# tarepan/ForwardTacotron

Measured on AMD Instinct MI355X. Metric: mel-frames/sec at batch=64 LJSpeech shapes (ForwardTacotron.generate, B*T_mel per s), higher is better.
Workload: dtype fp32; 1 GPU; c3: ForwardTacotron generate, batch=64 per GPU, phoneme lengths U{50..200}; global_batch=64, T_phonemes=200, T_mel=1368, parallelism=dp1

## Files before the change

### forwardtacotron_amd/csrc/gemm.hip

```cpp
#include "common.h"

namespace {

constexpr int BM = 128;
constexpr int BN = 128;
constexpr int BK = 16;
constexpr int LDS_STRIDE = 20;
constexpr int MAX_GROUPS = 16;

enum { EPI_CONV = 0, EPI_HIGHWAY = 1 };

struct GemmGroup {
  const float *w;
  const __bf16 *w3;
  const float *colscale;
  int Kpad;
  const float *bias;
  const float *scale;
  const float *shift;
  int N, k, pad, Ktot;
  int ycol0;
  int ntiles;
  int tile0;
};
// ... 654 lines not shown
  const int tid = threadIdx.x;
  const int lane = tid & 63, wave = tid >> 6;
  const int fr = lane & 15, fs = lane >> 4;

  const float *arow[2];
  int at[2];
  bool aok[2];
#pragma unroll
  for (int mi = 0; mi < 2; ++mi) {
    const int m = m0 + wave * 32 + mi * 16 + fr;
    aok[mi] = m < p.M;
    const int mm = aok[mi] ? m : 0;
    const int b = mm / p.To;
    at[mi] = mm - b * p.To;
    arow[mi] = p.x + (int64_t)b * p.T * p.x_stride;
  }
  int nk = (G.Ktot + X6_BK - 1) / X6_BK;
  int kc0 = 0;
  if (p.split > 1) {
    kc0 = blockIdx.y * p.kc_per;
    nk = min(nk - kc0, p.kc_per);
  }
  int kk = kc0 * X6_BK + 8 * fs, tj = kk / p.Cin, tc = kk - tj * p.Cin;
  struct ARaw {
    f32x4 v[2][2];
    f32x4 u[MAXPOOL ? 2 : 1][2];
    unsigned okm;
  };
  auto loadA = [&](ARaw &r) {
    const bool kok = kk < G.Ktot;
    unsigned okm = 0;
#pragma unroll
    for (int mi = 0; mi < 2; ++mi) {
      const int ts = at[mi] + tj - G.pad;
      const bool ok = kok && aok[mi] && ts >= 0 && ts < p.T;
      const float *src = arow[mi] + (int64_t)(ok ? ts : 0) * p.x_stride + (ok ? tc : 0);
      r.v[mi][0] = *(const f32x4 *)src;
      r.v[mi][1] = *(const f32x4 *)(src + 4);
      if constexpr (MAXPOOL) {
        const float *sp = src - ((ok && ts > 0) ? p.x_stride : 0);
        r.u[mi][0] = *(const f32x4 *)sp;
        r.u[mi][1] = *(const f32x4 *)(sp + 4);
      }
      okm |= (unsigned)ok << mi;
    }
    r.okm = okm;
    kk += X6_BK;
    tc += X6_BK;
#pragma unroll
    for (int w = 0; w < 2; ++w) {
      const bool wrap = tc >= p.Cin;
      tc -= wrap ? p.Cin : 0;
      tj += wrap;
    }
  };
  float amax = 0.f;
  auto splitA = [&](const ARaw &r, frag (&a)[2][H3 ? 2 : 3]) {
#pragma unroll
    for (int mi = 0; mi < 2; ++mi) {
      f32x4 v0 = r.v[mi][0], v1 = r.v[mi][1];
      if constexpr (MAXPOOL) {
        v0 = fmax4(v0, r.u[mi][0]);
        v1 = fmax4(v1, r.u[mi][1]);
      }
      const bool ok = (r.okm >> mi) & 1u;
      v0 = sel4(ok, v0);
      v1 = sel4(ok, v1);
      if constexpr (H3) {
        amax = fmaxf(amax, fmaxf(fmaxf(fabsf(v0.x), fabsf(v0.y)), fmaxf(fabsf(v0.z), fabsf(v0.w))));
        amax = fmaxf(amax, fmaxf(fmaxf(fabsf(v1.x), fabsf(v1.y)), fmaxf(fabsf(v1.z), fabsf(v1.w))));
        f16x4 l1, l2, h1, h2;
        split2h(v0, l1, l2);
        split2h(v1, h1, h2);
        a[mi][0] = __builtin_shufflevector(l1, h1, 0, 1, 2, 3, 4, 5, 6, 7);
        a[mi][1] = __builtin_shufflevector(l2, h2, 0, 1, 2, 3, 4, 5, 6, 7);
      } else {
        bf16x4 l1, l2, l3, h1, h2, h3;
        split3(v0, l1, l2, l3);
        split3(v1, h1, h2, h3);
        a[mi][0] = __builtin_shufflevector(l1, h1, 0, 1, 2, 3, 4, 5, 6, 7);
        a[mi][1] = __builtin_shufflevector(l2, h2, 0, 1, 2, 3, 4, 5, 6, 7);
        a[mi][2] = __builtin_shufflevector(l3, h3, 0, 1, 2, 3, 4, 5, 6, 7);
      }
    }
  };

  typedef unsigned u32x4 __attribute__((ext_vector_type(4)));
  const __bf16 *bsrc[6];
  int boff[6];
#pragma unroll
  for (int i = 0; i < 6; ++i) {
    const int idx = tid + 256 * i;
    const int pc = idx >> 9, rem = idx & 511, nl = rem >> 2, seg = rem & 3;
    const int n = n0 + nl < G.N ? n0 + nl : G.N - 1;
    bsrc[i] = G.w3 + ((int64_t)pc * G.N + n) * G.Kpad + kc0 * X6_BK + seg * 8;
    boff[i] = pc * X6_PIECE + nl * X6_STRIDE + seg * 8;
  }
  const int kb_last = (nk - 1) * X6_BK;
  int kb = 0;
  auto loadB = [&](u32x4 (&rb)[6]) {
    const int o = kb < kb_last ? kb : kb_last;
#pragma unroll
    for (int i = 0; i < 6; ++i) rb[i] = *(const u32x4 *)(bsrc[i] + o);
    kb += X6_BK;
  };
  auto storeB = [&](const u32x4 (&rb)[6], int buf) {
#pragma unroll
    for (int i = 0; i < 6; ++i) *(u32x4 *)(lds + buf * 3 * X6_PIECE + boff[i]) = rb[i];
  };

  f32x4 acc[2][8];
#pragma unroll
  for (int mi = 0; mi < 2; ++mi)
#pragma unroll
    for (int ni = 0; ni < 8; ++ni) acc[mi][ni] = (f32x4){0.f, 0.f, 0.f, 0.f};

  auto mfma_chunk = [&](const frag (&a)[2][H3 ? 2 : 3], int buf) {
    const __bf16 *cur = lds + buf * 3 * X6_PIECE;
#pragma unroll
    for (int ni = 0; ni < 8; ++ni) {
      frag b[3];
#pragma unroll
      for (int pc = 0; pc < 3; ++pc)
        b[pc] = *(const frag *)(cur + pc * X6_PIECE + (ni * 16 + fr) * X6_STRIDE + 8 * fs);
#pragma unroll
      for (int mi = 0; mi < 2; ++mi) {
        f32x4 c = acc[mi][ni];
        if constexpr (H3) {
          c = mma16(a[mi][1], b[2], c);
          c = mma16(a[mi][0], b[1], c);
          c = mma16(a[mi][0], b[0], c);
        } else {
          c = mma16(a[mi][2], b[0], c);
          c = mma16(a[mi][1], b[1], c);
          c = mma16(a[mi][0], b[2], c);
          c = mma16(a[mi][1], b[0], c);
          c = mma16(a[mi][0], b[1], c);
          c = mma16(a[mi][0], b[0], c);
        }
        acc[mi][ni] = c;
      }
    }
  };

  constexpr bool DEEP = H3;
  ARaw ra0, ra1;
  u32x4 rb[6];
  loadA(ra0);
  loadB(rb);
  if constexpr (DEEP) loadA(ra1);
  storeB(rb, 0);
  loadB(rb);
  __syncthreads();
  auto step = [&](int kc, ARaw &ras) {
    frag a[2][H3 ? 2 : 3];
    splitA(ras, a);
    loadA(ras);
    if (kc + 1 < nk) storeB(rb, (kc + 1) & 1);
    loadB(rb);
    mfma_chunk(a, kc & 1);
    __syncthreads();
  };
  for (int kc = 0; kc < nk; kc += 2) {
    step(kc, ra0);
    if (kc + 1 >= nk) break;
    step(kc + 1, DEEP ? ra1 : ra0);
  }

  if constexpr (H3) {
    bool bad = !(amax <= 65504.f);
#pragma unroll
    for (int ni = 0; ni < 8; ++ni) {
      const int col = n0 + ni * 16 + fr;
      const float cs = G.colscale[col < G.N ? col : G.N - 1];
#pragma unroll
      for (int mi = 0; mi < 2; ++mi)
#pragma unroll
        for (int i = 0; i < 4; ++i) {
          const int row = m0 + wave * 32 + mi * 16 + 4 * fs + i;
          bad |= col < G.N && row >= 0 && row < p.M && !__builtin_isfinite(acc[mi][ni][i]);
          acc[mi][ni][i] *= cs;
        }
    }
    if (bad && p.status) atomicOr(p.status, 1u);
  }

  const int er = 4 * fs;
  if (p.split > 1) {
    float *part = p.part + (size_t)blockIdx.y * p.M * G.N;
#pragma unroll
    for (int ni = 0; ni < 8; ++ni) {
      const int col = n0 + ni * 16 + fr;
      if (col >= G.N) continue;
#pragma unroll
      for (int mi = 0; mi < 2; ++mi)
#pragma unroll
        for (int i = 0; i < 4; ++i) {
          const int row = m0 + wave * 32 + mi * 16 + er + i;
          if (row < p.M) part[(size_t)row * G.N + col] = acc[mi][ni][i];
        }
    }
    return;
  }
  if constexpr (EPI == EPI_CONV) {
#pragma unroll
    for (int ni = 0; ni < 8; ++ni) {
      const int col = n0 + ni * 16 + fr;
      if (col >= G.N) continue;
      const float bias = G.bias ? G.bias[col] : 0.f;
      const float sc = G.scale ? G.scale[col] : 1.f;
      const float sh = G.scale ? G.shift[col] : 0.f;
#pragma unroll
      for (int mi = 0; mi < 2; ++mi)
#pragma unroll
        for (int i = 0; i < 4; ++i) {
          const int row = m0 + wave * 32 + mi * 16 + er + i;
          if (row >= p.M) continue;
          float v = acc[mi][ni][i];
          if (G.bias) v += bias;
          if (p.relu) v = fmaxf(v, 0.f);
          if (G.scale) v = v * sc + sh;
          if (p.residual) v += p.residual[(int64_t)row * p.res_stride + col];
          if (p.y) p.y[(int64_t)row * p.y_stride + G.ycol0 + col] = v;
          if (p.yt) {
            const int b = row / p.To, t = row - b * p.To;
            p.yt[((int64_t)b * p.yt_channels + G.ycol0 + col) * p.To + t] = v;
          }
        }
    }
  } else {
#pragma unroll
    for (int q = 0; q < 2; ++q)
#pragma unroll
      for (int h = 0; h < 2; ++h) {
        if (n0 + q * 64 >= G.N) continue;
        const int ni = 4 * q + h;
        const int col = n0 / 2 + q * 32 + h * 16 + fr;
        const float b1 = p.b1[col], b2 = p.b2[col];
#pragma unroll
        for (int mi = 0; mi < 2; ++mi)
#pragma unroll
          for (int i = 0; i < 4; ++i) {
            const int row = m0 + wave * 32 + mi * 16 + er + i;
            if (row >= p.M) continue;
            const float x1 = acc[mi][ni][i] + b1;
            const float x2 = acc[mi][ni + 2][i] + b2;
            const float g = ftmi_sigmoid(x2);
            const float xin = p.x[(int64_t)row * p.x_stride + col];
            p.y[(int64_t)row * p.y_stride + col] = highway_mix(g, x1, xin);
          }
      }
  }
}

constexpr int SL_BM = 256;
constexpr int SL_BN = 128;
constexpr int SL_MAXK = 16;
constexpr int SL_SR = SL_BM + SL_MAXK - 1;
constexpr int SL_P = 48;
constexpr int SL_ZROW = SL_SR;
constexpr int SL_AIMG = (SL_SR + 1) * SL_P;
constexpr int SL_BIMG = SL_BN * SL_P;
constexpr int SL_TP = SL_BN + 4;

__device__ __forceinline__ void slab_tile(int bid, int MT, int VT, int band, int &mt, int &v8) {
  if (MT < 8) {
    mt = bid % MT;
    v8 = bid / MT;
    return;
  }
  const int x = bid & 7, s8 = bid >> 3;
  if (band <= 0 || band >= VT) {
    const int q8 = s8 / VT;
    mt = q8 * 8 + x;
    v8 = s8 - q8 * VT;
    return;
  }
  const int MTx = (MT + 7) >> 3;
  const int per = MTx * band, b = s8 / per, rem = s8 - b * per;
  const int cbn = min(band, VT - b * band);
  const int lr = rem / cbn;
  mt = lr * 8 + x;
  v8 = b * band + (rem - lr * cbn);
  if (lr >= MTx) mt = MT;
}


template <int EPI, int NTHR>
__device__ __forceinline__ void slab_epilogue(const GemmParams &p, const GemmGroup &G,
                                              float *tile, int m0, int n0, int tid) {
  const int rows = min(SL_BM, p.M - m0);
  const int ncols = min(SL_BN, G.N - n0);

  if (p.split > 1) {
    float *part = p.part + (size_t)blockIdx.y * p.M * G.N;
    for (int idx = tid; idx < SL_BM * (SL_BN / 4); idx += NTHR) {
      const int r = idx >> 5, c = (idx & 31) * 4;
      if (r < rows && c < ncols)
        *(f32x4 *)(part + (size_t)(m0 + r) * G.N + n0 + c) = *(const f32x4 *)(tile + r * SL_TP + c);
    }
    return;
  }
  if constexpr (EPI == EPI_CONV) {
    if (p.pool_out) {
      for (int idx = tid; idx < SL_BM * (SL_BN / 4); idx += NTHR) {
        const int r = idx >> 5, c = (idx & 31) * 4;
        if (r >= rows || c >= ncols) continue;
        const int col = n0 + c;
        f32x4 v = *(const f32x4 *)(tile + r * SL_TP + c);
        if (G.bias) v += *(const f32x4 *)(G.bias + col);
        if (p.relu) v = fmax4(v, (f32x4){0.f, 0.f, 0.f, 0.f});
        if (G.scale) v = v * *(const f32x4 *)(G.scale + col) + *(const f32x4 *)(G.shift + col);
        *(f32x4 *)(tile + r * SL_TP + c) = v;
      }
      __syncthreads();
      float ymax = 0.f;
      for (int idx = tid; idx < SL_BM * (SL_BN / 4); idx += NTHR) {
        const int r = idx >> 5, c = (idx & 31) * 4;
        if (r == 0 || r >= rows || c >= ncols) continue;
        const int row = m0 + r, col = n0 + c;
        f32x4 v = *(const f32x4 *)(tile + r * SL_TP + c);
        if (row % p.T > 0) v = fmax4(v, *(const f32x4 *)(tile + (r - 1) * SL_TP + c));
        if (p.y_split_c) {
          ymax = fmaxf(ymax, fmaxf(fmaxf(fabsf(v.x), fabsf(v.y)), fmaxf(fabsf(v.z), fabsf(v.w))));
          f16x4 h, t;
          split2h(v, h, t);
          _Float16 *yr = (_Float16 *)(p.y + (int64_t)row * p.y_stride) + G.ycol0 + col;
          *(f16x4 *)yr = h;
          *(f16x4 *)(yr + p.y_split_c) = t;
        } else {
          *(f32x4 *)(p.y + (int64_t)row * p.y_stride + G.ycol0 + col) = v;
        }
      }
      if (!(ymax <= 65504.f) && p.status) atomicOr(p.status, 1u);
      return;
    }
    for (int idx = tid; idx < SL_BM * (SL_BN / 4); idx += NTHR) {
      const int r = idx >> 5, c = (idx & 31) * 4;
      if (r >= rows || c >= ncols) continue;
      const int row = m0 + r, col = n0 + c;
      f32x4 v = *(const f32x4 *)(tile + r * SL_TP + c);
      if (G.bias) v += *(const f32x4 *)(G.bias + col);
      if (p.relu) v = fmax4(v, (f32x4){0.f, 0.f, 0.f, 0.f});
      if (G.scale) v = v * *(const f32x4 *)(G.scale + col) + *(const f32x4 *)(G.shift + col);
      if (p.residual) v += *(const f32x4 *)(p.residual + (int64_t)row * p.res_stride + col);
      if (p.y) *(f32x4 *)(p.y + (int64_t)row * p.y_stride + G.ycol0 + col) = v;
      if (p.yt) *(f32x4 *)(tile + r * SL_TP + c) = v;
    }
    if (p.yt) {
      __syncthreads();
      for (int idx = tid; idx < SL_BM * SL_BN; idx += NTHR) {
        const int r = idx & (SL_BM - 1), c = idx / SL_BM;
        if (r >= rows || c >= ncols) continue;
        const int row = m0 + r, b = row / p.To, t = row - b * p.To;
        p.yt[((int64_t)b * p.yt_channels + G.ycol0 + n0 + c) * p.To + t] = tile[r * SL_TP + c];
      }
    }
  } else {
    for (int idx = tid; idx < SL_BM * (SL_BN / 8); idx += NTHR) {
      const int r = idx >> 4, o = (idx & 15) * 4, q = o >> 5, h = o & 31;
      if (r >= rows || q * 64 >= ncols) continue;
      const int row = m0 + r, col = n0 / 2 + o;
      const f32x4 x1 = *(const f32x4 *)(tile + r * SL_TP + q * 64 + h) + *(const f32x4 *)(p.b1 + col);
      const f32x4 x2 = *(const f32x4 *)(tile + r * SL_TP + q * 64 + 32 + h) + *(const f32x4 *)(p.b2 + col);
      const f32x4 xin = *(const f32x4 *)(p.x + (int64_t)row * p.x_stride + col);
      f32x4 out;
#pragma unroll
      for (int e = 0; e < 4; ++e) {
        const float g = ftmi_sigmoid(x2[e]);
        out[e] = highway_mix(g, x1[e], xin[e]);
      }
      *(f32x4 *)(p.y + (int64_t)row * p.y_stride + col) = out;
    }
  }
}

template <int EPI, bool MAXPOOL, bool WS>
__global__ __launch_bounds__(WS ? 768 : 512, 1) void conv_gemm_slab_kernel(const GemmParams p) {
  constexpr int NTHR = WS ? 768 : 512;
  constexpr int NSTG = WS ? 256 : 512;
  constexpr int SL_ASLOTS = (SL_SR * 8 + NSTG - 1) / NSTG;
  constexpr int SL_BSLOTS = 1024 / NSTG;
  __shared__ __attribute__((aligned(16))) _Float16 lds[2 * 2 * SL_AIMG + 2 * 2 * SL_BIMG];
  static_assert(SL_BM * SL_TP * 4 <= sizeof(lds), "epilogue tile");
  _Float16 *const lds_a = lds;
  _Float16 *const lds_b = lds + 2 * 2 * SL_AIMG;
  typedef unsigned u32x4 __attribute__((ext_vector_type(4)));
  typedef unsigned u32x2 __attribute__((ext_vector_type(2)));
  const int TS = p.pool_out ? SL_BM - 1 : SL_BM;
  const int MT = (p.M + TS - 1) / TS, NT = p.g[0].ntiles, VT = p.ngroups * NT;
  int mt, v8;
  slab_tile(blockIdx.x, MT, VT, p.band, mt, v8);
  const int gi = v8 / NT, nt = v8 - gi * NT;
  if (mt >= MT) return;
  const GemmGroup &G = p.g[gi];
  const int m0 = p.pool_out ? mt * TS - 1 : mt * SL_BM, n0 = nt * SL_BN;
  const int k = G.k, pad = G.pad, Cin = p.Cin;

  const int tid = threadIdx.x, lane = tid & 63, wave = tid >> 6;
  const int wm = wave & 3, wn = (wave >> 2) & 1;
  const int fr = lane & 15, fs = lane >> 4;
  const bool is_mma = !WS || wave < 8;
  const bool is_stg = !WS || wave >= 8;
  const int stid = WS ? tid - 512 : tid;
// ... 2420 lines not shown
#else
    if (q.T == q.M)
      hipLaunchKernelGGL((conv_gemm_skinny_kernel<false, true, 0, true>), grid, block, 0, s, q);
    else
      hipLaunchKernelGGL((conv_gemm_skinny_kernel<false, true>), grid, block, 0, s, q);
#endif
  } else {
    dim3 grid(MT * q.ngroups * NT, q.split), block(512);
    const bool nm = q.T == q.M;
    if (maxpool && nm)
      hipLaunchKernelGGL((conv_gemm_skinny_kernel<true, false, 0, true>), grid, block, 0, s, q);
    else if (maxpool)
      hipLaunchKernelGGL(conv_gemm_skinny_kernel<true>, grid, block, 0, s, q);
    else if (nm)
      hipLaunchKernelGGL((conv_gemm_skinny_kernel<false, false, 0, true>), grid, block, 0, s, q);
    else
      hipLaunchKernelGGL(conv_gemm_skinny_kernel<false>, grid, block, 0, s, q);
  }
  FTMI_CHECK_LAUNCH();
  if (q.force_part) {
    const int64_t n_el = (int64_t)q.M * (q.g[0].N / 2);
    const int eb = (int)((n_el + 255) / 256 < 2048 ? (n_el + 255) / 256 : 2048);
    hipLaunchKernelGGL(skinny_highway_finish_kernel, dim3(eb), dim3(256), 0, s, q);
    FTMI_CHECK_LAUNCH();
  } else if (q.split > 1) {
    const int64_t n_el = (int64_t)q.M * q.g[0].N;
    if (q.split >= 8) {
      const int eb = (int)((n_el + 63) / 64 < 2048 ? (n_el + 63) / 64 : 2048);
      hipLaunchKernelGGL(skinny_finish_kernel<4>, dim3(eb, q.ngroups), dim3(256), 0, s, q);
    } else {
      const int eb = (int)((n_el + 255) / 256 < 1024 ? (n_el + 255) / 256 : 1024);
      hipLaunchKernelGGL(skinny_finish_kernel<1>, dim3(eb, q.ngroups), dim3(256), 0, s, q);
    }
    FTMI_CHECK_LAUNCH();
  }
  return FTMI_OK;
}

static bool bank_halves_ok(const GemmParams &p) {
  if (p.M <= 0 || p.M > 128 || p.ngroups < 2 || p.ngroups % 2 || p.To != p.T) return false;
  if (p.Cin % 64 || p.Cin > 2 * BH_MAXCH * 32) return false;
  if (!p.y || p.yt || p.residual || p.x_split || p.pool_out || p.y_split_c) return false;
  if (!p.tile_cnt || !p.part || p.g[0].N % 16) return false;
  const int units = (p.ngroups / 2) * (p.g[0].N / 16);
  if (units % 8 || units * 8 > FTMI_BANK_COUNTERS) return false;
  for (int i = 0; i < p.ngroups; ++i)
    if (p.g[i].k != p.ngroups - i || p.g[i].N != p.g[0].N || !p.g[i].w3 || !p.g[i].colscale)
      return false;
  return true;
}

static int64_t bank_halves_floats(int M, int K, int N) {
  const int MI = M <= 64 ? 4 : 8;
  return (int64_t)(K / 2) * (N / 16) * 2 * (2 * MI * 64) * 4;
}

static int launch_bank_halves(const GemmParams &p, hipStream_t s) {
  const int units = (p.ngroups / 2) * (p.g[0].N / 16);
  const dim3 grid(2 * units), block(512);
  const int nch = p.Cin / 64;
  const bool prenet = p.ngroups == 16 && p.g[0].N == 256 && nch == 4;
#ifdef FTMI_DIAG
  const char *dg = getenv("FTMI_BANK_HALVES_DIAG");
  const int diag = dg && prenet && p.M > 64 ? atoi(dg) : 0;
  if (diag && p.wimg) {
    switch (diag) {
#define FTMI_BH_DIAG(D_)                                                                          \
  case D_:                                                                                        \
    hipLaunchKernelGGL((conv_bank_halves_kernel<8, 4, D_, 16, 16, true>), grid, block, 0, s, p);    \
    break;
      FTMI_BH_DIAG(1) FTMI_BH_DIAG(2) FTMI_BH_DIAG(3) FTMI_BH_DIAG(4) FTMI_BH_DIAG(16)
      FTMI_BH_DIAG(18) FTMI_BH_DIAG(32) FTMI_BH_DIAG(128) FTMI_BH_DIAG(256) FTMI_BH_DIAG(512)
#undef FTMI_BH_DIAG
      default:
        hipLaunchKernelGGL((conv_bank_halves_kernel<8, 4, 0, 16, 16, true>), grid, block, 0, s, p);
    }
    FTMI_CHECK_LAUNCH();
    return FTMI_OK;
  }
#endif
#define FTMI_BH_NCH(MI_, PK_)                                                                            \
  switch (nch) {                                                                                         \
    case 1: hipLaunchKernelGGL((conv_bank_halves_kernel<MI_, 1, 0, 0, 0, PK_>), grid, block, 0, s, p); break; \
    case 2: hipLaunchKernelGGL((conv_bank_halves_kernel<MI_, 2, 0, 0, 0, PK_>), grid, block, 0, s, p); break; \
    case 3: hipLaunchKernelGGL((conv_bank_halves_kernel<MI_, 3, 0, 0, 0, PK_>), grid, block, 0, s, p); break; \
    default: hipLaunchKernelGGL((conv_bank_halves_kernel<MI_, 4, 0, 0, 0, PK_>), grid, block, 0, s, p);       \
  }
  if (p.wimg) {
    if (p.M <= 64) {
      FTMI_BH_NCH(4, true)
    } else if (prenet && p.T == p.M) {
      hipLaunchKernelGGL((conv_bank_halves_kernel<8, 4, 0, 16, 16, true, true>), grid, block, 0, s, p);
    } else if (prenet) {
      hipLaunchKernelGGL((conv_bank_halves_kernel<8, 4, 0, 16, 16, true>), grid, block, 0, s, p);
    } else {
      FTMI_BH_NCH(8, true)
    }
  } else if (p.M <= 64) {
    FTMI_BH_NCH(4, false)
  } else if (prenet && p.T == p.M) {
    hipLaunchKernelGGL((conv_bank_halves_kernel<8, 4, 0, 16, 16, false, true>), grid, block, 0, s, p);
  } else if (prenet) {
    hipLaunchKernelGGL((conv_bank_halves_kernel<8, 4, 0, 16, 16>), grid, block, 0, s, p);
  } else {
    FTMI_BH_NCH(8, false)
  }
#undef FTMI_BH_NCH
  FTMI_CHECK_LAUNCH();
  return FTMI_OK;
}

constexpr int BW_MIN_BLOCKS = 512;
int64_t split_block_bytes(int64_t N, int64_t K, int mma);
static bool bank_walk_ok(const GemmParams &p) {
  const char *e = getenv("FTMI_BANK_WALK");
  if (e && atoi(e) == 0) return false;
  const int64_t blocks = (p.M + SL_BM - 2) / (SL_BM - 1) * ((p.g[0].N + SL_BN - 1) / SL_BN);
  if (!e && blocks < BW_MIN_BLOCKS) return false;
  if (!p.pool_out || p.x_split || p.residual || p.yt || !p.y || p.split_req > 1) return false;
  if (p.Cin <= 0 || p.Cin > BW_MAXCH * 32 || p.Cin % 16 || p.To != p.T || p.M <= 0) return false;
  if (p.T < 4 || p.ngroups < 2 || p.ngroups > BW_MAXK || p.g[0].N % SL_BN) return false;
  const int NG = p.ngroups, N = p.g[0].N;
  const GemmGroup &g1 = p.g[NG - 1];
  const char *blk = (const char *)p.g[0].w3;
  for (int i = 0; i < NG; ++i) {
    const GemmGroup &g = p.g[i];
    const int k = NG - i, kp = (k * p.Cin + 31) / 32 * 32;
    if (i > 0) blk -= split_block_bytes(N, (int64_t)k * p.Cin, 2);
    if (g.k != k || g.pad != k / 2 || g.N != N || g.Kpad != kp || g.ycol0 != (k - 1) * N)
      return false;
    if ((const char *)g.w3 != blk || (const char *)g.colscale != blk + (int64_t)6 * N * kp)
      return false;
    if (g.bias || (g.scale != (g1.scale ? g1.scale + (int64_t)(k - 1) * N : nullptr)) ||
        (g.shift != (g1.scale ? g1.shift + (int64_t)(k - 1) * N : nullptr)) || !g.shift != !g.scale)
      return false;
  }
  return true;
}

static int launch_bank_walk(const GemmParams &p, hipStream_t s) {
  GemmParams q = p;
  q.g[0].ntiles = (q.g[0].N + SL_BN - 1) / SL_BN;
#ifdef FTMI_DIAG
  const char *de = getenv("FTMI_SLAB_DIAG");
  q.diag = de ? atoi(de) : 0;
#endif
  const int MT = (q.M + SL_BM - 2) / (SL_BM - 1);
  const int nblk = (MT < 8 ? MT : (MT + 7) / 8 * 8) * q.g[0].ntiles;
  hipLaunchKernelGGL(conv_bank_walk_kernel, dim3(nblk), dim3(512), 0, s, q);
  FTMI_CHECK_LAUNCH();
  return FTMI_OK;
}

int launch(const GemmParams &p, int epi, bool maxpool, int nblocks, int mma, hipStream_t s) {
  if (nblocks <= 0) return FTMI_OK;
  dim3 grid(nblocks), block(256);
  bool presplit = (mma == 1 && x6_variant() != 3) || mma == 2;
  for (int i = 0; i < p.ngroups; ++i) presplit &= p.g[i].w3 != nullptr;
  if (mma == 2 && !presplit) return FTMI_E_ARG;
  if (p.pool_out) {
    GemmParams q = p;
    q.split_req = 0;
    q.part = nullptr;
    if (!(mma == 2 && presplit && epi == EPI_CONV && !maxpool && !p.residual && !p.yt &&
          p.y && slab_ok(q, epi)))
      return FTMI_E_UNSUPPORTED;
    if (bank_walk_ok(q)) return launch_bank_walk(q, s);
    return launch_slab(q, epi, false, s);
  }
  if (p.y_split_c) return FTMI_E_UNSUPPORTED;
  if (p.x_split) {
    if (!(mma == 2 && presplit && !maxpool && slab_ok(p, epi))) return FTMI_E_UNSUPPORTED;
    return launch_slab(p, epi, false, s);
  }
  if (mma == 2 && presplit && skinny_ok(p, epi)) return launch_skinny(p, epi, maxpool, s);
  if (p.ngroups > 1 && p.split_req > 1) {
    GemmParams q = p;
    q.split_req = 0;
    q.part = nullptr;
    return launch(q, epi, maxpool, nblocks, mma, s);
  }
  if (mma == 2 && slab_ok(p, epi)) return launch_slab(p, epi, maxpool, s);
  if (presplit) {
    dim3 g2(nblocks, p.split > 1 ? p.split : 1);
    if (mma == 2) {
      if (epi == EPI_HIGHWAY)
        hipLaunchKernelGGL((conv_gemm_x6b_kernel<EPI_HIGHWAY, false, true>), g2, block, 0, s, p);
      else if (maxpool)
        hipLaunchKernelGGL((conv_gemm_x6b_kernel<EPI_CONV, true, true>), g2, block, 0, s, p);
      else
        hipLaunchKernelGGL((conv_gemm_x6b_kernel<EPI_CONV, false, true>), g2, block, 0, s, p);
    } else {
      if (epi == EPI_HIGHWAY)
        hipLaunchKernelGGL((conv_gemm_x6b_kernel<EPI_HIGHWAY, false, false>), g2, block, 0, s, p);
      else if (maxpool)
        hipLaunchKernelGGL((conv_gemm_x6b_kernel<EPI_CONV, true, false>), g2, block, 0, s, p);
      else
        hipLaunchKernelGGL((conv_gemm_x6b_kernel<EPI_CONV, false, false>), g2, block, 0, s, p);
    }
    FTMI_CHECK_LAUNCH();
    if (p.split > 1) {
      const int64_t total = (int64_t)p.M * p.g[0].N;
      const int eb = (int)((total + 255) / 256 < 4096 ? (total + 255) / 256 : 4096);
      hipLaunchKernelGGL(splitk_epilogue_kernel, dim3(eb), block, 0, s, p);
      FTMI_CHECK_LAUNCH();
    }
    return FTMI_OK;
  }
  if (mma == 1 && x6_variant() == 2) {
    dim3 g2(nblocks, p.split > 1 ? p.split : 1);
    if (epi == EPI_HIGHWAY)
      hipLaunchKernelGGL((conv_gemm_x6p_kernel<EPI_HIGHWAY, false>), g2, block, 0, s, p);
    else if (maxpool)
      hipLaunchKernelGGL((conv_gemm_x6p_kernel<EPI_CONV, true>), g2, block, 0, s, p);
    else
      hipLaunchKernelGGL((conv_gemm_x6p_kernel<EPI_CONV, false>), g2, block, 0, s, p);
    FTMI_CHECK_LAUNCH();
    if (p.split > 1) {
      const int64_t total = (int64_t)p.M * p.g[0].N;
      const int eb = (int)((total + 255) / 256 < 4096 ? (total + 255) / 256 : 4096);
      hipLaunchKernelGGL(splitk_epilogue_kernel, dim3(eb), block, 0, s, p);
      FTMI_CHECK_LAUNCH();
    }
    return FTMI_OK;
  }
  if (mma == 1 && p.split > 1) {
    dim3 g2(nblocks, p.split);
    if (maxpool)
      hipLaunchKernelGGL((conv_gemm_x6_kernel<EPI_CONV, true>), g2, block, 0, s, p);
    else
      hipLaunchKernelGGL((conv_gemm_x6_kernel<EPI_CONV, false>), g2, block, 0, s, p);
    FTMI_CHECK_LAUNCH();
    const int64_t total = (int64_t)p.M * p.g[0].N;
    const int eb = (int)((total + 255) / 256 < 4096 ? (total + 255) / 256 : 4096);
    hipLaunchKernelGGL(splitk_epilogue_kernel, dim3(eb), block, 0, s, p);
    FTMI_CHECK_LAUNCH();
    return FTMI_OK;
  }
  if (mma == 1) {
    if (epi == EPI_HIGHWAY)
      hipLaunchKernelGGL((conv_gemm_x6_kernel<EPI_HIGHWAY, false>), grid, block, 0, s, p);
    else if (maxpool)
      hipLaunchKernelGGL((conv_gemm_x6_kernel<EPI_CONV, true>), grid, block, 0, s, p);
    else
      hipLaunchKernelGGL((conv_gemm_x6_kernel<EPI_CONV, false>), grid, block, 0, s, p);
    FTMI_CHECK_LAUNCH();
    return FTMI_OK;
  }
  if (epi == EPI_HIGHWAY)
    hipLaunchKernelGGL((conv_gemm_kernel<EPI_HIGHWAY, false>), grid, block, 0, s, p);
  else if (maxpool)
    hipLaunchKernelGGL((conv_gemm_kernel<EPI_CONV, true>), grid, block, 0, s, p);
  else
    hipLaunchKernelGGL((conv_gemm_kernel<EPI_CONV, false>), grid, block, 0, s, p);
  FTMI_CHECK_LAUNCH();
  return FTMI_OK;
}

int64_t split_block_bytes(int64_t N, int64_t K, int mma) {
  const int64_t planes = 3 * N * ((K + X6_BK - 1) / X6_BK * X6_BK) * 2;
  return mma == 2 ? planes + (4 * N + 15) / 16 * 16 : planes;
}

void set_split(GemmGroup &g, const void *block, int mma) {
  g.w3 = (const __bf16 *)block;
  g.colscale = (block && mma == 2) ? (const float *)((const char *)block + 3LL * g.N * g.Kpad * 2)
                                   : nullptr;
}

}

extern "C" int ftmi_conv1d(const ftmi_conv_args *a, ftmi_stream_t stream) {
  if (!a || !a->x || !a->w || (!a->y && !a->yt)) return FTMI_E_ARG;
  if (a->B <= 0 || a->T <= 0 || a->Cin <= 0 || a->N <= 0 || a->k <= 0) return FTMI_E_ARG;
  if (a->Cin % 16 != 0) return FTMI_E_SHAPE;
  if (a->mma < 0 || a->mma > 2) return FTMI_E_ARG;
  if (a->mma == 2 && !a->w_split) return FTMI_E_ARG;
  if (a->pad < 0 || a->pad >= a->k + a->T) return FTMI_E_SHAPE;
  if ((a->bn_scale == nullptr) != (a->bn_shift == nullptr)) return FTMI_E_ARG;
  if (!ftmi_aligned16(a->x) || !ftmi_aligned16(a->w) || (a->x_stride & 3)) return FTMI_E_ALIGN;
  if (a->w_split && !ftmi_aligned16(a->w_split)) return FTMI_E_ALIGN;
  const int To = a->T_out > 0 ? a->T_out : a->T;
  if ((int64_t)a->B * To > INT32_MAX) return FTMI_E_SHAPE;
  GemmParams p = {};
  p.x = a->x;
  p.x_stride = a->x_stride;
  p.B = a->B;
  p.T = a->T;
  p.To = To;
  p.Cin = a->Cin;
  p.M = a->B * To;
  p.relu = a->relu;
  p.ngroups = 1;
  p.residual = a->residual;
  p.res_stride = a->res_stride;
  p.y = a->y;
  p.y_stride = a->y_stride;
  p.yt = a->yt;
  p.yt_channels = a->N;
  p.status = a->status;
  p.x_split = a->x_split != 0;
  if (p.x_split && (a->mma != 2 || a->maxpool || a->x_stride < a->Cin))
    return FTMI_E_UNSUPPORTED;
  GemmGroup &g = p.g[0];
  g.w = a->w;
  g.Kpad = (a->k * a->Cin + X6_BK - 1) / X6_BK * X6_BK;
  g.bias = a->bias;
  g.scale = a->bn_scale;
  g.shift = a->bn_shift;
  g.N = a->N;
  g.k = a->k;
  g.pad = a->pad;
  g.Ktot = a->k * a->Cin;
  g.ycol0 = 0;
  g.ntiles = (a->N + BN - 1) / BN;
  g.tile0 = 0;
  set_split(g, a->w_split, a->mma);
  const int mtiles = (p.M + BM - 1) / BM;
  p.split = 1;
  if (a->split_k > 1) {
    if (a->mma == 0 || !a->split_ws) return FTMI_E_ARG;
    const int nkc = (g.Ktot + X6_BK - 1) / X6_BK;
    const int kc_per = (nkc + a->split_k - 1) / a->split_k;
    p.split = (nkc + kc_per - 1) / kc_per;
    p.kc_per = kc_per;
    p.split_req = a->split_k;
    p.part = a->split_ws;
  }
  return launch(p, EPI_CONV, a->maxpool != 0, mtiles * g.ntiles, a->mma, ftmi_hs(stream));
}

namespace {
int set_bank_groups(GemmParams &p, const float *w, const void *w_split, int K, int Cout, int mma,
                    const float *bn_scale, const float *bn_shift) {
  const int Cin = p.Cin;
// ... 492 lines not shown
```

Measured before the change: 11.43 million mel-frames/s.

## Add narrow-N pointwise GEMM kernel with deeper operand prefetch

Adds a specialized kernel for 1x1 convolutions whose output width is at most 80 columns, such as the mel projection. Each block covers a full 128-row tile with only N/16 column fragments and keeps three A chunks and two B chunks in flight. This avoids wasting a 128-wide N tile on narrow outputs and adds a fused transposed-output epilogue. It also adds diagnostic paths, compiled only under FTMI_DIAG, that can skip loads, MFMAs or barriers to probe bottlenecks.

Result: no change. 11.51 million mel-frames/s, median of 6 (+0.7%).

```diff
diff --git a/forwardtacotron_amd/csrc/gemm.hip b/forwardtacotron_amd/csrc/gemm.hip
--- a/forwardtacotron_amd/csrc/gemm.hip
+++ b/forwardtacotron_amd/csrc/gemm.hip
@@ -830,6 +830,18 @@
   storeB(rb, 0);
   loadB(rb);
   __syncthreads();
+#ifdef FTMI_DIAG
+  const int diag = p.diag;
+  auto step = [&](int kc, ARaw &ras) {
+    frag a[2][H3 ? 2 : 3];
+    splitA(ras, a);
+    if (!(diag & 4)) loadA(ras);
+    if (kc + 1 < nk) storeB(rb, (kc + 1) & 1);
+    loadB(rb);
+    if (!(diag & 2)) mfma_chunk(a, kc & 1);
+    if (!(diag & 1)) __syncthreads();
+  };
+#else
   auto step = [&](int kc, ARaw &ras) {
     frag a[2][H3 ? 2 : 3];
     splitA(ras, a);
@@ -839,6 +851,7 @@
     mfma_chunk(a, kc & 1);
     __syncthreads();
   };
+#endif
   for (int kc = 0; kc < nk; kc += 2) {
     step(kc, ra0);
     if (kc + 1 >= nk) break;
@@ -928,6 +941,203 @@
             p.y[(int64_t)row * p.y_stride + col] = highway_mix(g, x1, xin);
           }
       }
+  }
+}
+
+template <int NI, bool DG = false>
+__global__ __launch_bounds__(256, 3) void conv_gemm_narrow_kernel(const GemmParams p) {
+  constexpr int DA = 3;
+  constexpr int DB = 2;
+  constexpr int NR = NI * 16;
+  constexpr int PLANE = NR * X6_STRIDE;
+  constexpr int NB = (NR * 8 + 255) / 256;
+  __shared__ __attribute__((aligned(16))) _Float16 lds[2 * 2 * PLANE];
+
+  const GemmGroup &G = p.g[0];
+  const int m0 = blockIdx.x * BM;
+  const int tid = threadIdx.x;
+  const int lane = tid & 63, wave = tid >> 6;
+  const int fr = lane & 15, fs = lane >> 4;
+  const int nk = p.Cin / X6_BK;
+
+  unsigned aoff[2];
+  bool aok[2];
+#pragma unroll
+  for (int mi = 0; mi < 2; ++mi) {
+    const int m = m0 + wave * 32 + mi * 16 + fr;
+    aok[mi] = m < p.M;
+    aoff[mi] = (unsigned)(aok[mi] ? m : 0) * (unsigned)p.x_stride + 8 * fs;
+  }
+  struct ARaw {
+    f32x4 v[2][2];
+  };
+  int ka = 0;
+  auto loadA = [&](ARaw &r) {
+    const unsigned o = (ka < nk ? ka : nk - 1) * X6_BK;
+#pragma unroll
+    for (int mi = 0; mi < 2; ++mi) {
+      r.v[mi][0] = *(const f32x4 *)(p.x + (aoff[mi] + o));
+      r.v[mi][1] = *(const f32x4 *)(p.x + (aoff[mi] + o + 4));
+    }
+    ++ka;
+  };
+  float amax = 0.f;
+  auto splitA = [&](const ARaw &r, f16x8 (&a)[2][2]) {
+#pragma unroll
+    for (int mi = 0; mi < 2; ++mi) {
+      const f32x4 v0 = sel4(aok[mi], r.v[mi][0]);
+      const f32x4 v1 = sel4(aok[mi], r.v[mi][1]);
+      amax = fmaxf(amax, fmaxf(fmaxf(fabsf(v0.x), fabsf(v0.y)), fmaxf(fabsf(v0.z), fabsf(v0.w))));
+      amax = fmaxf(amax, fmaxf(fmaxf(fabsf(v1.x), fabsf(v1.y)), fmaxf(fabsf(v1.z), fabsf(v1.w))));
+      f16x4 l1, l2, h1, h2;
+      split2h(v0, l1, l2);
+      split2h(v1, h1, h2);
+      a[mi][0] = __builtin_shufflevector(l1, h1, 0, 1, 2, 3, 4, 5, 6, 7);
+      a[mi][1] = __builtin_shufflevector(l2, h2, 0, 1, 2, 3, 4, 5, 6, 7);
+    }
+  };
+
+  typedef unsigned u32x4 __attribute__((ext_vector_type(4)));
+  const _Float16 *w16 = (const _Float16 *)G.w3;
+  unsigned bsrc[NB];
+  int boff[NB];
+  bool bok[NB];
+#pragma unroll
+  for (int i = 0; i < NB; ++i) {
+    const int idx = tid + 256 * i;
+    bok[i] = idx < NR * 8;
+    const int id = bok[i] ? idx : 0;
+    const int pc = id / (NR * 4), rem = id - pc * (NR * 4), nl = rem >> 2, seg = rem & 3;
+    bsrc[i] = (unsigned)(pc * NR + nl) * (unsigned)G.Kpad + seg * 8;
+    boff[i] = pc * PLANE + nl * X6_STRIDE + seg * 8;
+  }
+  int kb = 0;
+  auto loadB = [&](u32x4 (&rb)[NB]) {
+    const unsigned o = (kb < nk ? kb : nk - 1) * X6_BK;
+#pragma unroll
+    for (int i = 0; i < NB; ++i) rb[i] = *(const u32x4 *)(w16 + (bsrc[i] + o));
+    ++kb;
+  };
+  auto storeB = [&](const u32x4 (&rb)[NB], int buf) {
+#pragma unroll
+    for (int i = 0; i < NB; ++i)
+      if (256 * i + 255 < NR * 8 || bok[i]) *(u32x4 *)(lds + buf * 2 * PLANE + boff[i]) = rb[i];
+  };
+
+  f32x4 acc[2][NI];
+#pragma unroll
+  for (int mi = 0; mi < 2; ++mi)
+#pragma unroll
+    for (int ni = 0; ni < NI; ++ni) acc[mi][ni] = (f32x4){0.f, 0.f, 0.f, 0.f};
+
+  auto mfma_chunk = [&](const f16x8 (&a)[2][2], int buf) {
+    const _Float16 *cur = lds + buf * 2 * PLANE + fr * X6_STRIDE + 8 * fs;
+#pragma unroll
+    for (int ni = 0; ni < NI; ++ni) {
+      const f16x8 b0 = *(const f16x8 *)(cur + ni * 16 * X6_STRIDE);
+      const f16x8 b1 = *(const f16x8 *)(cur + PLANE + ni * 16 * X6_STRIDE);
+      const f16x8 bh = b0 * (_Float16)(1.0f / H3_SCALE);
+#pragma unroll
+      for (int mi = 0; mi < 2; ++mi) {
+        f32x4 c = acc[mi][ni];
+        c = mma16(a[mi][1], bh, c);
+        c = mma16(a[mi][0], b1, c);
+        c = mma16(a[mi][0], b0, c);
+        acc[mi][ni] = c;
+      }
+    }
+  };
+
+  ARaw ra[DA];
+  u32x4 rb[DB][NB];
+  static_assert(DA == DB + 1, "the prologue loads weight chunks 0 .. DA - 1");
+  loadA(ra[0]);
+  loadB(rb[0]);
+  storeB(rb[0], 0);
+#pragma unroll
+  for (int j = 1; j < DA; ++j) {
+    loadB(rb[j % DB]);
+    loadA(ra[j]);
+  }
+  __syncthreads();
+#ifdef FTMI_DIAG
+  const int diag = DG ? p.diag : 0;
+#else
+  constexpr int diag = 0;
+#endif
+  auto step = [&](int kc, ARaw &ras, u32x4 (&rbs)[NB]) {
+    f16x8 a[2][2];
+    splitA(ras, a);
+    if (!(diag & 8)) {
+      storeB(rbs, (kc + 1) & 1);
+      loadB(rbs);
+    }
+    if (!(diag & 4)) loadA(ras);
+    if (!(diag & 2)) mfma_chunk(a, kc & 1);
+    if (!(diag & 1)) __syncthreads();
+  };
+  constexpr int U = DA * DB;
+  for (int kc = 0;; kc += U) {
+#pragma unroll
+    for (int u = 0; u < U; ++u) {
+      step(kc + u, ra[u % DA], rb[(u + 1) % DB]);
+      if (kc + u + 1 >= nk) goto done;
+    }
+  }
+done:;
+
+  bool bad = !(amax <= 65504.f);
+#pragma unroll
+  for (int ni = 0; ni < NI; ++ni) {
+    const float cs = G.colscale[ni * 16 + fr];
+#pragma unroll
+    for (int mi = 0; mi < 2; ++mi)
+#pragma unroll
+      for (int i = 0; i < 4; ++i) {
+        const int row = m0 + wave * 32 + mi * 16 + 4 * fs + i;
+        bad |= row < p.M && !__builtin_isfinite(acc[mi][ni][i]);
+        acc[mi][ni][i] *= cs;
+      }
+  }
+  if (bad && p.status) atomicOr(p.status, 1u);
+
+  const bool yt16 = p.yt && (((uintptr_t)p.yt & 15u) == 0);
+#pragma unroll
+  for (int mi = 0; mi < 2; ++mi) {
+    const int row0 = m0 + wave * 32 + mi * 16 + 4 * fs;
+    if (row0 >= p.M) continue;
+    const int b0 = row0 / p.To, t0 = row0 - b0 * p.To;
+#pragma unroll
+    for (int ni = 0; ni < NI; ++ni) {
+      const int col = ni * 16 + fr;
+      const float bias = G.bias ? G.bias[col] : 0.f;
+      f32x4 v = acc[mi][ni];
+#pragma unroll
+      for (int i = 0; i < 4; ++i) {
+        const int row = row0 + i;
+        if (row >= p.M) continue;
+        float e = v[i];
+        if (G.bias) e += bias;
+        if (p.relu) e = fmaxf(e, 0.f);
+        if (p.residual) e += p.residual[(int64_t)row * p.res_stride + col];
+        if (p.y) p.y[(int64_t)row * p.y_stride + col] = e;
+        v[i] = e;
+      }
+      if (p.yt) {
+        const int64_t o = ((int64_t)b0 * p.yt_channels + col) * p.To + t0;
+        if (yt16 && row0 + 3 < p.M && t0 + 3 < p.To && (o & 3) == 0) {
+          *(f32x4 *)(p.yt + o) = v;
+        } else {
+#pragma unroll
+          for (int i = 0; i < 4; ++i) {
+            const int row = row0 + i;
+            if (row >= p.M) continue;
+            const int b = row / p.To, t = row - b * p.To;
+            p.yt[((int64_t)b * p.yt_channels + col) * p.To + t] = v[i];
+          }
+        }
+      }
+    }
   }
 }
 
@@ -3654,6 +3864,41 @@
   return FTMI_OK;
 }
 
+static bool narrow_ok(const GemmParams &p, int epi, bool maxpool) {
+  const char *e = getenv("FTMI_GEMM_NARROW");
+  if (e && atoi(e) == 0) return false;
+  const GemmGroup &g = p.g[0];
+  return epi == EPI_CONV && !maxpool && p.ngroups == 1 && g.k == 1 && g.pad == 0 && p.To == p.T &&
+         g.N % 16 == 0 && g.N <= 80 && p.Cin % 32 == 0 && g.Kpad == p.Cin && p.split <= 1 &&
+         !g.scale && g.ycol0 == 0 && p.x_stride >= p.Cin &&
+         (int64_t)p.M * p.x_stride < ((int64_t)1 << 31);
+}
+
+static int launch_narrow(const GemmParams &p, hipStream_t s) {
+  dim3 grid((p.M + BM - 1) / BM), block(256);
+#ifdef FTMI_DIAG
+  {
+    const char *de = getenv("FTMI_NARROW_DIAG");
+    GemmParams q = p;
+    q.diag = de ? atoi(de) : 0;
+    if (p.g[0].N == 80 && q.diag) {
+      hipLaunchKernelGGL((conv_gemm_narrow_kernel<5, true>), grid, block, 0, s, q);
+      FTMI_CHECK_LAUNCH();
+      return FTMI_OK;
+    }
+  }
+#endif
+  switch (p.g[0].N / 16) {
+    case 1: hipLaunchKernelGGL(conv_gemm_narrow_kernel<1>, grid, block, 0, s, p); break;
+    case 2: hipLaunchKernelGGL(conv_gemm_narrow_kernel<2>, grid, block, 0, s, p); break;
+    case 3: hipLaunchKernelGGL(conv_gemm_narrow_kernel<3>, grid, block, 0, s, p); break;
+    case 4: hipLaunchKernelGGL(conv_gemm_narrow_kernel<4>, grid, block, 0, s, p); break;
+    default: hipLaunchKernelGGL(conv_gemm_narrow_kernel<5>, grid, block, 0, s, p); break;
+  }
+  FTMI_CHECK_LAUNCH();
+  return FTMI_OK;
+}
+
 int launch(const GemmParams &p, int epi, bool maxpool, int nblocks, int mma, hipStream_t s) {
   if (nblocks <= 0) return FTMI_OK;
   dim3 grid(nblocks), block(256);
@@ -3683,6 +3928,21 @@
     return launch(q, epi, maxpool, nblocks, mma, s);
   }
   if (mma == 2 && slab_ok(p, epi)) return launch_slab(p, epi, maxpool, s);
+  if (mma == 2 && narrow_ok(p, epi, maxpool)) return launch_narrow(p, s);
+#ifdef FTMI_DIAG
+  if (presplit && mma == 2 && epi == EPI_CONV && !maxpool) {
+    const char *de = getenv("FTMI_X6B_DIAG");
+    if (de && atoi(de)) {
+      GemmParams q = p;
+      q.diag = atoi(de);
+      q.status = nullptr;
+      hipLaunchKernelGGL((conv_gemm_x6b_kernel<EPI_CONV, false, true>),
+                         dim3(nblocks, p.split > 1 ? p.split : 1), block, 0, s, q);
+      FTMI_CHECK_LAUNCH();
+      return FTMI_OK;
+    }
+  }
+#endif
   if (presplit) {
     dim3 g2(nblocks, p.split > 1 ? p.split : 1);
     if (mma == 2) {
```
